# LUMII-Syslab/DiffusionSAT

Measured on NVIDIA B200. Metric: diffusion samples/sec, 3-SAT n=100, higher is better.
Workload: dtype f32

## Files before the change

### diffusionsat_b200/csrc/dsat_api.cu

```cuda
#include <cuda_runtime.h>
#include <math.h>
#include <stdint.h>
#include <stdio.h>
#include <stdlib.h>
#include <string.h>

#include <algorithm>
#include <string>
#include <type_traits>
#include <vector>

#include "../../include/dsat.h"
#include "../../include/dsat_debug.h"
#include "dsat_common.cuh"
#include "dsat_gemm_simt.cuh"
#include "dsat_message.cuh"
#include "dsat_spmm.cuh"
#include "dsat_graph_host.cuh"
#include "dsat_norm_head.cuh"
#include "dsat_hist.cuh"
#include "dsat_gemm_tc.cuh"
#include "dsat_mlp_fused.cuh"
#include "dsat_mlp_x3.cuh"

// ... 434 lines not shown
    cudaEventRecord(c->prof[c->prof_used].ev, c->stream);
    c->prof_used++;
}

int x3_pack_weights(dsat_ctx* c) {
    struct Cut { int op, col0, n; };
    const Cut cuts[12] = {
        {OP_V1, 0, c->HQ}, {OP_Q2, 0, c->Q}, {OP_V1, c->HQ, c->HL}, {OP_L2, 0, c->HL}, {OP_L3, 0, 2 * c->Q},
        {OP_C1, 0, c->HC}, {OP_C2, 0, c->Q + c->F}, {OP_U1, 0, c->HU}, {OP_U2, 0, c->HU}, {OP_U3, 0, c->F},
        {OP_O1, 0, c->HO}, {OP_O2, 0, DSAT_LOGIT_PAD}};
    for (int i = 0; i < 12; ++i) {
        const int op = cuts[i].op, K = c->ops[op].K, Nop = c->ops[op].N, n = cuts[i].n;
        const int K64 = (K + 63) / 64 * 64;
        std::vector<float> w((size_t)K * Nop);
        CK_CUDA(c, dsat_memcpy_sync(w.data(), c->ops[op].w.p, w.size() * sizeof(float), cudaMemcpyDeviceToHost));
        std::vector<__nv_bfloat16> wt((size_t)2 * n * K64, __float2bfloat16(0.f));
        for (int k = 0; k < K; ++k)
            for (int j = 0; j < n; ++j) {
                const float v = w[(size_t)k * Nop + cuts[i].col0 + j];
                const __nv_bfloat16 hi = __float2bfloat16(v);
                wt[(size_t)j * K64 + k] = hi;
                wt[(size_t)(n + j) * K64 + k] = __float2bfloat16(v - __bfloat162float(hi));
            }
        CK_CUDA(c, c->wx[i].alloc(wt.size()));
        CK_CUDA(c, dsat_memcpy_sync(c->wx[i].p, wt.data(), wt.size() * 2, cudaMemcpyHostToDevice));
        c->wx_k64[i] = K64; c->wx_n[i] = n;
    }
    return DSAT_OK;
}

enum { XQ = 0, XL1, XL2, XL3, XC, XU, XO };

int ensure_x3_buffers(dsat_ctx* c) {
    if (c->has_x3_buffers) return DSAT_OK;
    int rc = ensure_common_buffers(c);
    if (rc) return rc;
    const size_t Nt = (size_t)c->Nt, Mt = (size_t)c->Mt;
    const int F = c->F, Q = c->Q;
    CK_CUDA(c, c->VROWp.alloc(2 * Nt * c->ldv()));
    CK_CUDA(c, c->CROWp.alloc(2 * Mt * c->ldc()));
    CK_CUDA(c, c->SPREp.alloc(2 * Nt * F));
    CK_CUDA(c, c->H1p.alloc(2 * Nt * c->HL));
    CK_CUDA(c, c->H2p.alloc(2 * Nt * c->HL));
    CK_CUDA(c, cudaMemsetAsync(c->VROWp.p, 0, c->VROWp.count * 2, c->stream));
    CK_CUDA(c, cudaMemsetAsync(c->CROWp.p, 0, c->CROWp.count * 2, c->stream));
    struct L { int wi; int op; int bias_off; int epi; };
    auto build = [&](int which, const __nv_bfloat16* a_hi, size_t a_plane, long long rows, int k, int lda,
                     std::initializer_list<L> layers, int n_groups, int out_mode, void* out0, void* out1, int ld_out) -> bool {
        x3::X3Mlp& f = c->x3[which];
        f.ready = false;
        x3::X3Params& p = f.p;
        p.n_layers = (int)layers.size();
        p.rows = (int)rows;
        p.n_groups = n_groups;
        p.a_box_rows = (int)(rows < x3::BLOCK_M ? rows : x3::BLOCK_M);
        p.qmaps = Q;
        p.prof = nullptr;
        p.out_mode = out_mode; p.out0 = out0; p.out1 = out1; p.ld_out = ld_out;
        {
            const SkipInfo sk = skip_info(c);
            p.done = sk.done; p.chains_per_group = sk.chains_per_group;
            p.rows_per_chain = rows == c->Mt ? c->m : c->n;
        }
        f.pair_mode = which != XQ && which != XO;
        if (!tc::make_bf16_map(&f.map_a_hi, a_hi, rows, k, lda, p.a_box_rows)) return false;
        if (!tc::make_bf16_map(&f.map_a_lo, a_hi + a_plane, rows, k, lda, p.a_box_rows)) return false;
        int i = 0;
        for (const L& l : layers) {
            x3::X3Layer& ly = p.layer[i];
            const int n_total = c->wx_n[l.wi];
            ly.K = c->ops[l.op].K; ly.N = n_groups > 1 ? 256 : n_total; ly.n_total = n_total;
            ly.epi = l.epi; ly.w_lo_row = n_total; ly.bias = c->ops[l.op].b.p + l.bias_off;
            if (n_groups > 1 && n_total != 256 * n_groups) return false;
            ++i;
        }
        if (!x3::plan_x3(f)) return false;
        i = 0;
        for (const L& l : layers) {
            const int box = f.p.pair ? p.layer[i].N / 2 : p.layer[i].N;
            if (!tc::make_bf16_map(&f.map_w[i], c->wx[l.wi].p, 2 * c->wx_n[l.wi], c->wx_k64[l.wi], c->wx_k64[l.wi], box)) return false;
            ++i;
        }
        for (; i < x3::MAX_LAYERS; ++i) f.map_w[i] = f.map_w[0];
        if (getenv("DSAT_PLAN_LOG"))
            fprintf(stderr, "[dsat] x3 mlp %d: smem %d B, input ring %d, weight ring %d x %d B, epilogue warps %d, cta pair %d, groups %d\n",
                    which, f.smem_bytes, p.a_slots, p.w_slots, p.w_slot_bytes, p.epi_warps, p.pair, p.n_groups);
        return true;
    };
    const size_t vplane = Nt * c->ldv(), cplane = Mt * c->ldc(), splane = Nt * F, hplane = Nt * c->HL;
    bool ok = true;
    ok = ok && build(XQ, c->VROWp.p, vplane, c->Nt, F + DSAT_AUX_PAD, c->ldv(),
                     {{0, OP_V1, 0, tc::TC_LRELU}, {1, OP_Q2, 0, tc::TC_QUERY}}, 1, x3::OUT_F32, c->QS.p, nullptr, 3 * Q);
    const int lgroups = c->HL > 256 ? c->HL / 256 : 1;
    ok = ok && (c->HL <= 256 || c->HL % 256 == 0);
    ok = ok && build(XL1, c->VROWp.p, vplane, c->Nt, F + DSAT_AUX_PAD, c->ldv(),
                     {{2, OP_V1, c->HQ, tc::TC_LRELU}}, lgroups, x3::OUT_SPLIT, c->H1p.p, c->H1p.p + hplane, c->HL);
    ok = ok && build(XL2, c->H1p.p, hplane, c->Nt, c->HL, c->HL,
                     {{3, OP_L2, 0, tc::TC_LRELU}}, lgroups, x3::OUT_SPLIT, c->H2p.p, c->H2p.p + hplane, c->HL);
    const int l3groups = 2 * Q > 256 ? 2 * Q / 256 : 1;
    ok = ok && build(XL3, c->H2p.p, hplane, c->Nt, c->HL, c->HL,
                     {{4, OP_L3, 0, tc::TC_LINEAR}}, l3groups, x3::OUT_F32, c->LIT.p, nullptr, 2 * Q);
    if (Q + F <= 256 && c->HC <= 256)
        ok = ok && build(XC, c->CROWp.p, cplane, c->Mt, F + 2 * Q, c->ldc(),
                         {{5, OP_C1, 0, tc::TC_LRELU}, {6, OP_C2, 0, tc::TC_LINEAR}}, 1, x3::OUT_F32, c->COUT.p, nullptr, Q + F);
    else ok = false;
    if (c->HU <= 256)
        ok = ok && build(XU, c->VROWp.p, vplane, c->Nt, F + DSAT_AUX_PAD + 3 * Q, c->ldv(),
                         {{7, OP_U1, 0, tc::TC_LRELU}, {8, OP_U2, 0, tc::TC_LRELU}, {9, OP_U3, 0, tc::TC_LINEAR}}, 1, x3::OUT_F32,
                         c->UOUT.p, nullptr, F);
    else ok = false;
    ok = ok && build(XO, c->SPREp.p, splane, c->Nt, F, F,
                     {{10, OP_O1, 0, tc::TC_LRELU}, {11, OP_O2, 0, tc::TC_LINEAR}}, 1, x3::OUT_F32, c->LOGITS.p, nullptr, DSAT_LOGIT_PAD);
    c->x3_ready = ok;
    if (!ok) { c->err = "the fp32-accurate tensor-core path supports feature_maps = query_maps <= 128 (hidden widths <= 256 or 512)"; return DSAT_ERR_UNSUPPORTED; }
    c->has_x3_buffers = true;
    return DSAT_OK;
}

int run_x3(dsat_ctx* c, int which, int prof_class) {
    prof_mark(c, prof_class);
    CK_CUDA(c, x3::launch_x3(c->x3[which], c->device, c->sm_count, c->stream));
    c->launches++;
    return DSAT_OK;
}

int run_linear(dsat_ctx* c, int op, const float* A, int lda, float* Y, int ldy, long long rows, int epi) {
    prof_mark(c, op);
    LinearOp l;
    l.A = A; l.lda = lda; l.W = c->ops[op].w.p; l.ldw = c->ops[op].N; l.bias = c->ops[op].b.p;
    l.Y = Y; l.ldy = ldy; l.rows = (int)rows; l.K = c->ops[op].K; l.N = c->ops[op].N; l.epi = epi; l.qmaps = c->Q;
    CK_CUDA(c, launch_sgemm(l, c->stream));
    c->launches++;
    return DSAT_OK;
}

template <typename KernelLauncher>
int dispatch_width(dsat_ctx* c, int width, KernelLauncher&& fn) {
    switch (width) {
        case 64: fn(std::integral_constant<int, 2>()); break;
        case 128: fn(std::integral_constant<int, 4>()); break;
        case 256: fn(std::integral_constant<int, 8>()); break;
        default: c->err = "feature width must be 64, 128 or 256"; return DSAT_ERR_UNSUPPORTED;
    }
    return DSAT_OK;
}

struct LossScalars { float t, ts, norm_plus; };


float kl_host(float pa, float pb) {
    float qa = 1.0f - pa;
    float t1 = pa == 0.f ? 0.f : pa * (logf(pa) - logf(pb));
    float t2 = qa == 0.f ? 0.f : qa * (log1pf(-pa) - log1pf(-pb));
    return t1 + t2;
}
LossScalars loss_scalars(float noise_scale) {
    LossScalars s;
    s.t = powf(noise_scale, 0.5f);
    s.ts = fminf(s.t + 0.01f, 1.0f);
    float pa = 0.0f * (1.0f - s.ts) + s.ts / 2.0f;
    float pb = 0.0f * (1.0f - 1.0f) + 1.0f / 2.0f;
    s.norm_plus = kl_host(pa, pb) + 1e-4f;
    return s;
}

static inline bool use_tc(const dsat_ctx* c) { return c->precision == DSAT_BF16 || c->precision == DSAT_BF16_UNFUSED; }
static inline bool use_x3(const dsat_ctx* c) { return c->precision == DSAT_F32_TC; }
static inline float* vrow_f(dsat_ctx* c) { return c->precision == DSAT_F32 ? c->VROW.p : nullptr; }
static inline __nv_bfloat16* vrow_b(dsat_ctx* c) { return use_tc(c) ? c->VROWb.p : use_x3(c) ? c->VROWp.p : nullptr; }
// ... 1432 lines not shown
```

### diffusionsat_b200/csrc/dsat_gemm_tc.cuh

```cuda
#pragma once
#include <cuda.h>
#include "dsat_common.cuh"

namespace dsat {
namespace tc {

constexpr int BLOCK_M = 128;
constexpr int BLOCK_N = 256;
constexpr int BLOCK_K = 64;
constexpr int STAGES = 2;
constexpr int THREADS = 192;
constexpr int A_BYTES = BLOCK_M * BLOCK_K * 2;
constexpr int B_BYTES = BLOCK_N * BLOCK_K * 2;
constexpr int SMEM_BYTES = STAGES * (A_BYTES + B_BYTES) + 1024  + 256 ;

enum TcEpilogue : int { TC_LINEAR = 0, TC_LRELU = 1, TC_QUERY = 2 };

struct TcOut {
    void* ptr0; int ld0; int bf16_0;
    void* ptr1; int ld1; int bf16_1;
    int split;
};

__device__ __forceinline__ uint32_t smem_u32(const void* p) { return (uint32_t)__cvta_generic_to_shared(p); }
// ... 340 lines not shown
        }
    } else {
        const int quad = warp & 3;
        const size_t row = (size_t)row0 + quad * 32 + lane;
        mbar_wait(tmem_full_bar, 0);
        tcgen05_fence_after();
        for (int c = 0; c < bn; c += 32) {
            uint32_t raw[32];
            tmem_ld_32cols(tmem_base + ((uint32_t)(quad * 32) << 16) + (uint32_t)c, raw);
            if (row < (size_t)rows) {
                float v[32];
                const int col = n0 + c;
#pragma unroll
                for (int j = 0; j < 32; ++j) {
                    float x = __uint_as_float(raw[j]) + ((col + j < N) ? __ldg(bias + col + j) : 0.f);
                    if (epi == TC_LRELU) x = x > 0.f ? x : 0.2f * x;
                    v[j] = x;
                }
                const int valid = min(32, bn - c);
                if (valid == 32) {
                    store_chunk(out, row, col, v);
                    if (epi == TC_QUERY) {
                        float sp[32], sn[32];
#pragma unroll
                        for (int j = 0; j < 32; ++j) {
                            const float tail = __logf(1.0f + __expf(-fabsf(v[j])));
                            sp[j] = fmaxf(v[j], 0.f) + tail;
                            sn[j] = fmaxf(-v[j], 0.f) + tail;
                        }
                        store_chunk(out, row, col + qmaps, sp);
                        store_chunk(out, row, col + 2 * qmaps, sn);
                    }
                } else {
                    const bool second = out.ptr1 != nullptr && col >= out.split;
                    void* base = second ? out.ptr1 : out.ptr0;
                    const int ld = second ? out.ld1 : out.ld0;
                    const int cc = second ? col - out.split : col;
                    const int is_bf16 = second ? out.bf16_1 : out.bf16_0;
                    for (int j = 0; j < valid; ++j) {
                        if (is_bf16) reinterpret_cast<__nv_bfloat16*>(base)[row * ld + cc + j] = __float2bfloat16_rn(v[j]);
                        else reinterpret_cast<float*>(base)[row * ld + cc + j] = v[j];
                    }
                }
            }
        }
        tcgen05_fence_before();
    }
    __syncthreads();
    if (warp == 1) {
        tcgen05_fence_after();
        asm volatile("tcgen05.dealloc.cta_group::1.sync.aligned.b32 %0, %1;" ::"r"(tmem_base), "n"(BLOCK_N));
    }
}

typedef CUresult (*EncodeTiledFn)(CUtensorMap*, CUtensorMapDataType, cuuint32_t, void*, const cuuint64_t*,
                                  const cuuint64_t*, const cuuint32_t*, const cuuint32_t*, CUtensorMapInterleave,
                                  CUtensorMapSwizzle, CUtensorMapL2promotion, CUtensorMapFloatOOBfill);

inline EncodeTiledFn encode_tiled_fn() {
    static EncodeTiledFn fn = nullptr;
    if (!fn) {
        void* p = nullptr;
        cudaDriverEntryPointQueryResult q;
        if (cudaGetDriverEntryPoint("cuTensorMapEncodeTiled", &p, cudaEnableDefault, &q) == cudaSuccess &&
            q == cudaDriverEntryPointSuccess)
            fn = reinterpret_cast<EncodeTiledFn>(p);
    }
    return fn;
}

inline bool make_bf16_map(CUtensorMap* map, const void* base, long long rows, int cols, int ld, int box_rows) {
    EncodeTiledFn fn = encode_tiled_fn();
    if (!fn) return false;
    cuuint64_t dims[2] = {(cuuint64_t)cols, (cuuint64_t)rows};
    cuuint64_t strides[1] = {(cuuint64_t)ld * 2};
    cuuint32_t box[2] = {(cuuint32_t)BLOCK_K, (cuuint32_t)box_rows};
    cuuint32_t estr[2] = {1, 1};
    CUresult r = fn(map, CU_TENSOR_MAP_DATA_TYPE_BFLOAT16, 2, const_cast<void*>(base), dims, strides, box, estr,
                    CU_TENSOR_MAP_INTERLEAVE_NONE, CU_TENSOR_MAP_SWIZZLE_128B, CU_TENSOR_MAP_L2_PROMOTION_L2_256B,
                    CU_TENSOR_MAP_FLOAT_OOB_FILL_NONE);
    return r == CUDA_SUCCESS;
}

struct TcLinear {
    CUtensorMap map_a, map_b;
    const float* bias;
    TcOut out;
    int rows, K, N, epi, qmaps;
    int a_box_rows, b_box_rows;
};

inline cudaError_t configure_tc_device() {
    static PerDeviceOnce configured;
    if (configured.done()) return cudaSuccess;
    cudaError_t e = cudaFuncSetAttribute(tc_linear_kernel, cudaFuncAttributeMaxDynamicSharedMemorySize, SMEM_BYTES);
    if (e == cudaSuccess) configured.mark();
    return e;
}

inline cudaError_t launch_tc_linear(const TcLinear& op, cudaStream_t stream) {
    if (op.rows <= 0) return cudaSuccess;
    {
        cudaError_t e = configure_tc_device();
        if (e != cudaSuccess) return e;
    }
    const int n_tiles = ceil_div(op.N, BLOCK_N);
    const unsigned grid = (unsigned)(n_tiles * ceil_div(op.rows, BLOCK_M));
    tc_linear_kernel<<<grid, THREADS, SMEM_BYTES, stream>>>(op.map_a, op.map_b, op.bias, op.out, op.rows, op.K, op.N,
                                                             n_tiles, op.epi, op.qmaps, op.a_box_rows, op.b_box_rows);
    return cudaGetLastError();
}

}
}
```

### diffusionsat_b200/csrc/dsat_mlp_x3.cuh

```cuda
#pragma once
#include "dsat_mlp_fused.cuh"

namespace dsat {
namespace x3 {

constexpr int BLOCK_M = 128;
constexpr int BLOCK_K = 64;
constexpr int BLK_BYTES = BLOCK_M * BLOCK_K * 2;
constexpr int MAX_LAYERS = 3;
constexpr int MAX_RING = 12;
constexpr int TMEM_COLS = 512;
constexpr int STAGE_ROW = 128 + 16;
constexpr int SKIP_UNITS = 1024;
constexpr int SKIP_OFF = 512;
constexpr int BAR_BYTES = SKIP_OFF + SKIP_UNITS / 8;
static_assert((4 * MAX_RING + 6) * 8 + 4 <= SKIP_OFF, "x3 barriers overlap the early-exit bits");
constexpr int SMEM_LIMIT = 227 * 1024;

enum OutMode : int { OUT_F32 = 0, OUT_SPLIT = 1 };

struct X3Layer {
    int K, N;
    int epi;
    int w_lo_row;
    int bias_off;
    int n_total;
    const float* bias;
};

struct X3Params {
    int n_layers;
    X3Layer layer[MAX_LAYERS];
    int rows, n_tiles, n_groups, a_box_rows;
    int a_slots, w_slots, w_slot_bytes;
    int epi_warps, smem_pad, bias_total, qmaps, pair;
    int out_mode;
    void* out0; void* out1; int ld_out;
    long long* prof;
    const int* done; int rows_per_chain, chains_per_group;
};

__device__ __forceinline__ void split2(float v0, float v1, uint32_t& hi, uint32_t& lo) { split_bf16x2(v0, v1, hi, lo); }

struct Epi {
    uint32_t lane_addr, bl_addr, stage_addr;
    int N, epi, cpar, cstep, lane, qmaps, col0;
    size_t row_first; int rows_left;
    void* out0; void* out1; int ld_out, out_mode;
};

__device__ __forceinline__ void epi_hidden(const Epi& e, const uint32_t (&raw)[32], int c) {
    float v[32];
    fm::bias_act_chunk(raw, e.bl_addr + 4u * (uint32_t)c, e.epi == tc::TC_LRELU, v);
    uint32_t w[32];
#pragma unroll
    for (int i = 0; i < 16; ++i) split2(v[2 * i], v[2 * i + 1], w[i], w[16 + i]);
    fm::tmem_st_32cols(e.lane_addr + (uint32_t)c, w);
}

__device__ __forceinline__ void epi_final(const Epi& e, const uint32_t (&raw)[32], int c) {
    float v[32];
    fm::bias_act_chunk(raw, e.bl_addr + 4u * (uint32_t)c, e.epi == tc::TC_LRELU, v);
    const int valid = min(32, e.N - c);
    const int col = e.col0 + c;
    if (e.out_mode == OUT_SPLIT) {
        uint4 hi[4], lo[4];
#pragma unroll
        for (int q = 0; q < 4; ++q) {
            split2(v[8 * q], v[8 * q + 1], hi[q].x, lo[q].x);
            split2(v[8 * q + 2], v[8 * q + 3], hi[q].y, lo[q].y);
            split2(v[8 * q + 4], v[8 * q + 5], hi[q].z, lo[q].z);
            split2(v[8 * q + 6], v[8 * q + 7], hi[q].w, lo[q].w);
        }
        const size_t pitch = (size_t)e.ld_out * 2;
        fm::store_chunk_packed(e.stage_addr, STAGE_ROW, e.lane, hi, valid, reinterpret_cast<uint8_t*>(e.out0), pitch, e.row_first, e.rows_left, col);
        fm::store_chunk_packed(e.stage_addr, STAGE_ROW, e.lane, lo, valid, reinterpret_cast<uint8_t*>(e.out1), pitch, e.row_first, e.rows_left, col);
        return;
    }
    uint8_t* gbase = reinterpret_cast<uint8_t*>(e.out0);
    const size_t pitch = (size_t)e.ld_out * 4;
    fm::store_chunk_fast<false>(e.stage_addr, STAGE_ROW, e.lane, v, valid, gbase, pitch, e.row_first, e.rows_left, col);
    if (e.epi == tc::TC_QUERY) {
        float sp[32], sn[32];
#pragma unroll
        for (int i = 0; i < 32; ++i) {
            const float t = __logf(1.0f + __expf(-fabsf(v[i])));
            sp[i] = fmaxf(v[i], 0.f) + t;
            sn[i] = fmaxf(-v[i], 0.f) + t;
        }
        fm::store_chunk_fast<false>(e.stage_addr, STAGE_ROW, e.lane, sp, valid, gbase, pitch, e.row_first, e.rows_left, col + e.qmaps);
        fm::store_chunk_fast<false>(e.stage_addr, STAGE_ROW, e.lane, sn, valid, gbase, pitch, e.row_first, e.rows_left, col + 2 * e.qmaps);
    }
}

template <bool PAIR>
__global__ void __launch_bounds__(64 + 32 * 8, 1)
x3_mlp_kernel(const __grid_constant__ CUtensorMap map_a_hi, const __grid_constant__ CUtensorMap map_a_lo,
              const __grid_constant__ CUtensorMap map_w0, const __grid_constant__ CUtensorMap map_w1,
              const __grid_constant__ CUtensorMap map_w2, X3Params p) {
    using namespace tc;
    extern __shared__ __align__(1024) uint8_t smem_raw[];
    uint8_t* smem = reinterpret_cast<uint8_t*>((reinterpret_cast<uintptr_t>(smem_raw) + 1023) & ~(uintptr_t)1023);
    if ((int)(smem - smem_raw) > p.smem_pad) __trap();
    uint8_t* a_ring = smem;
    uint8_t* w_ring = a_ring + (size_t)p.a_slots * BLK_BYTES;
    uint8_t* stage_all = w_ring + (size_t)p.w_slots * p.w_slot_bytes;
    uint8_t* tail = stage_all + (size_t)p.epi_warps * 32 * STAGE_ROW;
    uint64_t* a_full = reinterpret_cast<uint64_t*>(tail);
    uint64_t* a_empty = a_full + MAX_RING;
    uint64_t* w_full = a_empty + MAX_RING;
    uint64_t* w_empty = w_full + MAX_RING;
    uint64_t* tmem_full = w_empty + MAX_RING;
    uint64_t* tmem_empty = tmem_full + 2;
    uint64_t* h_full = tmem_empty + 2;
    uint32_t* tmem_slot = reinterpret_cast<uint32_t*>(h_full + 2);
    float* bias_s = reinterpret_cast<float*>(tail + BAR_BYTES);

    const int warp = threadIdx.x >> 5, lane = threadIdx.x & 31;
    const int epi_threads = 32 * p.epi_warps;
    const CUtensorMap* map_w[MAX_LAYERS] = {&map_w0, &map_w1, &map_w2};
    const CUtensorMap* map_a[2] = {&map_a_hi, &map_a_lo};
    const uint32_t rank = PAIR ? cluster_rank() : 0u;
    const bool leader = rank == 0;
    constexpr int NC = PAIR ? 2 : 1;
    const bool timing = p.prof != nullptr && blockIdx.x == 0;

    if (threadIdx.x == 0) {
        for (int s = 0; s < MAX_RING; ++s) {
            mbar_init(&a_full[s], NC); mbar_init(&a_empty[s], 1);
            mbar_init(&w_full[s], NC); mbar_init(&w_empty[s], 1);
        }
        for (int b = 0; b < 2; ++b) { mbar_init(&tmem_full[b], 1); mbar_init(&tmem_empty[b], NC * p.epi_warps); }
        for (int h = 0; h < 2; ++h) mbar_init(&h_full[h], NC * p.epi_warps);
        asm volatile("fence.mbarrier_init.release.cluster;" ::: "memory");
        asm volatile("prefetch.tensormap [%0];" ::"l"(&map_a_hi) : "memory");
        asm volatile("prefetch.tensormap [%0];" ::"l"(&map_a_lo) : "memory");
        asm volatile("prefetch.tensormap [%0];" ::"l"(&map_w0) : "memory");
        asm volatile("prefetch.tensormap [%0];" ::"l"(&map_w1) : "memory");
        asm volatile("prefetch.tensormap [%0];" ::"l"(&map_w2) : "memory");
    }
    if (warp == 1) {
        if constexpr (PAIR) {
            asm volatile("tcgen05.alloc.cta_group::2.sync.aligned.shared::cta.b32 [%0], %1;" ::"r"(smem_u32(tmem_slot)), "n"(TMEM_COLS));
            asm volatile("tcgen05.relinquish_alloc_permit.cta_group::2.sync.aligned;");
        } else {
            asm volatile("tcgen05.alloc.cta_group::1.sync.aligned.shared::cta.b32 [%0], %1;" ::"r"(smem_u32(tmem_slot)), "n"(TMEM_COLS));
            asm volatile("tcgen05.relinquish_alloc_permit.cta_group::1.sync.aligned;");
        }
    }
    if (warp >= 2 && warp < 2 + p.epi_warps) {
        for (int l = 0; l < p.n_layers; ++l)
            for (int i = threadIdx.x - 64; i < p.layer[l].n_total; i += epi_threads) bias_s[p.layer[l].bias_off + i] = __ldg(p.layer[l].bias + i);
    }
    tcgen05_fence_before();
    __syncthreads();
    if constexpr (PAIR) cluster_sync_all();
    tcgen05_fence_after();
    const uint32_t tmem_base = *tmem_slot;
    const int L = p.n_layers, G = p.n_groups;
    auto at_leader = [&](uint64_t* bar) -> uint32_t { return PAIR ? mapa_rank(smem_u32(bar), 0) : smem_u32(bar); };
    const int unit0 = PAIR ? (int)(blockIdx.x >> 1) : (int)blockIdx.x;
    const int unit_stride = PAIR ? (int)(gridDim.x >> 1) : (int)gridDim.x;
    const int n_units = (PAIR ? (p.n_tiles + 1) / 2 : p.n_tiles) * G;
    const int nt = unit0 < n_units ? (n_units - unit0 + unit_stride - 1) / unit_stride : 0;
    auto tile_of = [&](int j) { const int u = (unit0 + j * unit_stride) / G; return PAIR ? 2 * u + (int)rank : u; };
    auto group_of = [&](int j) { return (unit0 + j * unit_stride) % G; };
    uint32_t* skip_bits = reinterpret_cast<uint32_t*>(tail + SKIP_OFF);
    const bool skipping = p.done != nullptr && nt <= SKIP_UNITS;
    if (skipping) {
        for (int base = 32 * warp; base < nt; base += (int)blockDim.x) {
            const int j = base + lane;
            bool all = false;
            if (j < nt) {
                const int u = (unit0 + j * unit_stride) / G;
                const int r0 = (PAIR ? 2 * u : u) * BLOCK_M;
                int r1 = r0 + (PAIR ? 2 * BLOCK_M : BLOCK_M);
                r1 = (r1 < p.rows ? r1 : p.rows) - 1;
                const int g0 = (r0 / p.rows_per_chain) / p.chains_per_group, g1 = (r1 / p.rows_per_chain) / p.chains_per_group;
                all = true;
                for (int g = g0; g <= g1 && all; ++g) all = __ldg(p.done + g) != 0;
            }
            const uint32_t bits = __ballot_sync(0xffffffffu, all);
// ... 71 lines not shown
                    }
                } else {
                    for (int k = 0; k < ksteps; ++k) {
                        if constexpr (PAIR) umma_bf16_elect_cg2(acc, da + (uint64_t)(2 * k), db + (uint64_t)(2 * k), idesc, (accum | (uint32_t)k) != 0);
                        else umma_bf16_elect(acc, da + (uint64_t)(2 * k), db + (uint64_t)(2 * k), idesc, (accum | (uint32_t)k) != 0);
                    }
                    if (free_bar) commit(free_bar);
                }
            };
#define X3_WAIT(acc_t, call) do { if (timing) { const long long t0__ = clock64(); call; acc_t += clock64() - t0__; } else { call; } } while (0)
            int jp = 0;
            for (int j = 0; j < nt; ++j) {
                if (unit_done(j)) continue;
                for (int l = 0; l < L; ++l) {
                    const int g = jp * L + l, buf = g & 1, use = g >> 1;
                    X3_WAIT(t_wait_acc, mbar_wait(&tmem_empty[buf], (uint32_t)((use & 1) ^ 1)));
                    if (g > 0 && (l > 0 ? l - 1 : L - 1) > 0)
                        X3_WAIT(t_wait_read, mbar_wait(&tmem_full[buf ^ 1], (uint32_t)(((g - 1) >> 1) & 1)));
                    const uint32_t h_par = (uint32_t)((jp * (L - 1) + (l - 1)) & 1);
                    tcgen05_fence_after();
                    const int K = p.layer[l].K, N = p.layer[l].N;
                    const int kbs = (K + BLOCK_K - 1) / BLOCK_K;
                    const uint32_t idesc = make_idesc_bf16(PAIR ? 2 * BLOCK_M : BLOCK_M, N);
                    const uint32_t acc = tmem_base + (uint32_t)(buf * 256);
                    const uint32_t hid = tmem_base + (uint32_t)((buf ^ 1) * 256);
                    for (int kb = 0; kb < kbs; ++kb) {
                        const int ksteps = min(BLOCK_K / 16, (K - kb * BLOCK_K + 15) / 16);
                        if (l == 0) {
                            const int as_hi = as;
                            const uint32_t ph_hi = aph;
                            if (++as == p.a_slots) { as = 0; aph ^= 1; }
                            const int as_lo = as;
                            const uint32_t ph_lo = aph;
                            if (++as == p.a_slots) { as = 0; aph ^= 1; }
                            X3_WAIT(t_wait_a, mbar_wait(&a_full[as_hi], ph_hi));
                            X3_WAIT(t_wait_a, mbar_wait(&a_full[as_lo], ph_lo));
                            const uint64_t da_hi = make_smem_desc_sw128(smem_u32(a_ring + (size_t)as_hi * BLK_BYTES));
                            const uint64_t da_lo = make_smem_desc_sw128(smem_u32(a_ring + (size_t)as_lo * BLK_BYTES));
                            X3_WAIT(t_wait_w, mbar_wait(&w_full[ws], wph));
                            uint64_t db = make_smem_desc_sw128(smem_u32(w_ring + (size_t)ws * p.w_slot_bytes));
                            kblock(acc, da_hi, db, idesc, kb != 0, ksteps, nullptr);
                            kblock(acc, da_lo, db, idesc, 1u, ksteps, &w_empty[ws]);
                            if (++ws == p.w_slots) { ws = 0; wph ^= 1; }
                            X3_WAIT(t_wait_w, mbar_wait(&w_full[ws], wph));
                            db = make_smem_desc_sw128(smem_u32(w_ring + (size_t)ws * p.w_slot_bytes));
                            kblock(acc, da_hi, db, idesc, 1u, ksteps, &w_empty[ws]);
                            if (++ws == p.w_slots) { ws = 0; wph ^= 1; }
                            commit(&a_empty[as_hi]); commit(&a_empty[as_lo]);
                        } else {
                            const uint32_t ta_hi = hid + (uint32_t)(kb * BLOCK_K), ta_lo = ta_hi + 16;
                            if ((kb & 1) == 0 && kb < 4) {
                                X3_WAIT(t_wait_h, mbar_wait(&h_full[kb >> 1], h_par));
                                tcgen05_fence_after();
                            }
                            X3_WAIT(t_wait_w, mbar_wait(&w_full[ws], wph));
                            uint64_t db = make_smem_desc_sw128(smem_u32(w_ring + (size_t)ws * p.w_slot_bytes));
                            kblock_ts(acc, ta_hi, db, idesc, kb != 0, ksteps, nullptr);
                            kblock_ts(acc, ta_lo, db, idesc, 1u, ksteps, &w_empty[ws]);
                            if (++ws == p.w_slots) { ws = 0; wph ^= 1; }
                            X3_WAIT(t_wait_w, mbar_wait(&w_full[ws], wph));
                            db = make_smem_desc_sw128(smem_u32(w_ring + (size_t)ws * p.w_slot_bytes));
                            kblock_ts(acc, ta_hi, db, idesc, 1u, ksteps, &w_empty[ws]);
                            if (++ws == p.w_slots) { ws = 0; wph ^= 1; }
                        }
                    }
                    commit(&tmem_full[buf]);
                }
                ++jp;
            }
#undef X3_WAIT
            if (timing && lane == 0) {
                p.prof[0] = clock64() - t_begin; p.prof[1] = t_wait_acc; p.prof[2] = t_wait_h; p.prof[3] = t_wait_a; p.prof[4] = t_wait_w;
                p.prof[8] = t_wait_read;
            }
        }
    } else if (warp < 2 + p.epi_warps) {
        const int quad = warp & 3;
        Epi e;
        e.lane = lane;
        e.cpar = (warp - 2) >> 2;
        e.cstep = 32 * (p.epi_warps >> 2);
        e.qmaps = p.qmaps;
        e.out0 = p.out0; e.out1 = p.out1; e.ld_out = p.ld_out; e.out_mode = p.out_mode;
        const uint32_t bias_addr0 = smem_u32(bias_s);
        e.stage_addr = smem_u32(stage_all) + (uint32_t)(warp - 2) * (32 * STAGE_ROW);
        long long t_wait_full = 0, t_hidden = 0, t_final = 0;
        int jp = -1;
        for (int j = 0; j < nt; ++j) {
            if (unit_done(j)) continue;
            ++jp;
            const int tile = tile_of(j), grp = group_of(j);
            DSAT_CHECK(tile >= 0 && (tile < p.n_tiles || (PAIR && tile == p.n_tiles)) && grp >= 0 && grp < G);
            e.row_first = (size_t)tile * BLOCK_M + quad * 32;
            e.rows_left = p.rows - (int)e.row_first;
            e.col0 = grp * 256;
            for (int l = 0; l < L; ++l) {
                const int g = jp * L + l, buf = g & 1, use = g >> 1;
                e.N = p.layer[l].N; e.epi = p.layer[l].epi;
                e.bl_addr = bias_addr0 + 4u * (uint32_t)(p.layer[l].bias_off + grp * 256);
                e.lane_addr = tmem_base + ((uint32_t)(quad * 32) << 16) + (uint32_t)(buf * 256);
                const long long t0 = timing ? clock64() : 0;
                mbar_wait(&tmem_full[buf], (uint32_t)(use & 1));
                tcgen05_fence_after();
                const long long t1 = timing ? clock64() : 0;
                const uint32_t empty_addr = at_leader(&tmem_empty[buf]);
                if (l + 1 < L) {
                    bool low_done = false;
                    auto release = [&](int h) {
                        fm::tmem_st_wait();
                        tcgen05_fence_before();
                        __syncwarp();
                        if (lane == 0) {
                            if (h == 1) fm::arrive_addr<PAIR>(empty_addr);
                            fm::arrive_addr<PAIR>(at_leader(&h_full[h]));
                        }
                    };
                    int c = 32 * e.cpar;
                    if (c < e.N) {
                        uint32_t ra[32], rb[32];
                        fm::tmem_ld_32cols_async(e.lane_addr + (uint32_t)c, ra);
#pragma unroll 1
                        while (true) {
                            fm::tmem_ld_wait(ra);
                            const int c1 = c + e.cstep;
                            if (c1 < e.N) fm::tmem_ld_32cols_async(e.lane_addr + (uint32_t)c1, rb);
                            epi_hidden(e, ra, c);
                            if (!low_done && c1 >= 128) { release(0); low_done = true; }
                            if (c1 >= e.N) break;
                            fm::tmem_ld_wait(rb);
                            c = c1 + e.cstep;
                            if (c < e.N) fm::tmem_ld_32cols_async(e.lane_addr + (uint32_t)c, ra);
                            epi_hidden(e, rb, c1);
                            if (!low_done && c >= 128) { release(0); low_done = true; }
                            if (c >= e.N) break;
                        }
                    }
                    if (!low_done) release(0);
                    release(1);
                    if (timing) t_hidden += clock64() - t1;
                } else {
                    bool released = false;
#pragma unroll 1
                    for (int c = 32 * e.cpar; c < e.N; c += e.cstep) {
                        uint32_t ra[32];
                        fm::tmem_ld_32cols_async(e.lane_addr + (uint32_t)c, ra);
                        fm::tmem_ld_wait(ra);
                        if (c + e.cstep >= e.N) {
                            tcgen05_fence_before();
                            fm::warp_arrive<PAIR>(empty_addr, lane);
                            released = true;
                        }
                        epi_final(e, ra, c);
                    }
                    if (!released) { tcgen05_fence_before(); fm::warp_arrive<PAIR>(empty_addr, lane); }
                    if (timing) t_final += clock64() - t1;
                }
                if (timing) t_wait_full += t1 - t0;
            }
        }
        if (timing && warp == 2 && lane == 0) { p.prof[5] = t_wait_full; p.prof[6] = t_hidden; p.prof[7] = t_final; }
    }
    tcgen05_fence_before();
    __syncthreads();
    if constexpr (PAIR) cluster_sync_all();
    if (warp == 1) {
        tcgen05_fence_after();
        if constexpr (PAIR) asm volatile("tcgen05.dealloc.cta_group::2.sync.aligned.b32 %0, %1;" ::"r"(tmem_base), "n"(TMEM_COLS));
        else asm volatile("tcgen05.dealloc.cta_group::1.sync.aligned.b32 %0, %1;" ::"r"(tmem_base), "n"(TMEM_COLS));
    }
}

struct X3Mlp {
    CUtensorMap map_a_hi, map_a_lo;
    CUtensorMap map_w[MAX_LAYERS];
    X3Params p;
    int smem_bytes = 0;
    bool pair_mode = false;
    bool ready = false;
};

inline bool plan_x3(X3Mlp& f) {
    X3Params& p = f.p;
    const int pad = fm::dyn_smem_pad();
    p.smem_pad = pad;
    int bias_total = 0, max_n = 0;
    bool pair = f.pair_mode && p.rows > BLOCK_M;
    for (int l = 0; l < p.n_layers; ++l) {
        X3Layer& ly = p.layer[l];
        if (ly.N > 256 || ly.N % 16 || ly.K % 16) return false;
        if (l > 0 && ly.K > p.layer[l - 1].N) return false;
        ly.bias_off = bias_total;
        bias_total += (ly.n_total + 31) / 32 * 32;
        max_n = max(max_n, ly.N);
    }
    if (p.n_groups > 1 && p.n_layers != 1) return false;
    p.pair = pair ? 1 : 0;
    p.bias_total = bias_total;
    p.n_tiles = ceil_div(p.rows, BLOCK_M);
    p.w_slot_bytes = ((pair ? max_n / 2 : max_n) * BLOCK_K * 2 + 1023) / 1024 * 1024;
    for (int ew : {8, 4}) {
        const int fixed = pad + ew * 32 * STAGE_ROW + BAR_BYTES + bias_total * 4;
        int avail = SMEM_LIMIT - fixed;
        int a = 2, w = 2;
        if (avail < a * BLK_BYTES + w * p.w_slot_bytes) continue;
        avail -= a * BLK_BYTES + w * p.w_slot_bytes;
        while (true) {
            bool grew = false;
            if (a <= w && a < MAX_RING && avail >= BLK_BYTES) { ++a; avail -= BLK_BYTES; grew = true; }
            else if (w < MAX_RING && avail >= p.w_slot_bytes) { ++w; avail -= p.w_slot_bytes; grew = true; }
            else if (a < MAX_RING && avail >= BLK_BYTES) { ++a; avail -= BLK_BYTES; grew = true; }
            if (!grew) break;
        }
        p.a_slots = a; p.w_slots = w; p.epi_warps = ew;
        f.smem_bytes = fixed + a * BLK_BYTES + w * p.w_slot_bytes;
        f.ready = true;
        return true;
    }
    return false;
}

inline cudaError_t configure_x3_device(int) {
    static PerDeviceOnce configured;
    if (configured.done()) return cudaSuccess;
    cudaError_t e = cudaFuncSetAttribute(x3_mlp_kernel<false>, cudaFuncAttributeMaxDynamicSharedMemorySize, SMEM_LIMIT);
    if (e == cudaSuccess) e = cudaFuncSetAttribute(x3_mlp_kernel<true>, cudaFuncAttributeMaxDynamicSharedMemorySize, SMEM_LIMIT);
    if (e == cudaSuccess) configured.mark();
    return e;
}

inline cudaError_t launch_x3(const X3Mlp& f, int device, int sm_count, cudaStream_t stream) {
    if (f.p.rows <= 0) return cudaSuccess;
    cudaError_t e = configure_x3_device(device);
    if (e != cudaSuccess) return e;
    const unsigned threads = 64 + 32 * f.p.epi_warps;
    if (f.p.pair) {
        const int n_units = (f.p.n_tiles + 1) / 2 * f.p.n_groups;
        const int pairs = n_units < sm_count / 2 ? n_units : sm_count / 2;
        cudaLaunchConfig_t cfg = {};
        cfg.gridDim = dim3(2 * pairs); cfg.blockDim = dim3(threads); cfg.dynamicSmemBytes = (size_t)f.smem_bytes; cfg.stream = stream;
        cudaLaunchAttribute attr[1];
        attr[0].id = cudaLaunchAttributeClusterDimension;
        attr[0].val.clusterDim.x = 2; attr[0].val.clusterDim.y = 1; attr[0].val.clusterDim.z = 1;
        cfg.attrs = attr; cfg.numAttrs = 1;
        return cudaLaunchKernelEx(&cfg, x3_mlp_kernel<true>, f.map_a_hi, f.map_a_lo, f.map_w[0], f.map_w[1], f.map_w[2], f.p);
    }
    const int n_units = f.p.n_tiles * f.p.n_groups;
    const unsigned grid = (unsigned)(n_units < sm_count ? n_units : sm_count);
    x3_mlp_kernel<false><<<grid, threads, f.smem_bytes, stream>>>(f.map_a_hi, f.map_a_lo, f.map_w[0], f.map_w[1], f.map_w[2], f.p);
    return cudaGetLastError();
}

}
}
```

### diffusionsat_b200/csrc/dsat_norm_head.cuh

```cuda
#pragma once
#include "dsat_common.cuh"
#include "dsat_message.cuh"

namespace dsat {

template <int V>
__device__ __forceinline__ int lane_col(int lane, int i) {
    if constexpr (V == 2) return lane * 2 + i;
    else return (i >> 2) * 128 + lane * 4 + (i & 3);
}

constexpr int PN_WARPS = 8;
#ifndef PN_BF16_CTAS
#define PN_BF16_CTAS 4
#endif
constexpr int PN_UNROLL = 4;

template <int V, typename TS, typename TX>
__global__ void __launch_bounds__(PN_WARPS * 32)
pairnorm_kernel(const int* __restrict__ seg, int n_graphs_unit, int rows_per_chain, int total_graphs,
                const TS* __restrict__ SRC, int ld_src, int src_off,
                TX* __restrict__ STATE, int ld_state,
                TX* __restrict__ PRE, int ld_pre,
                __nv_bfloat16* STATE_HI = nullptr, size_t state_plane = 0,
// ... 17 lines not shown
            for (; r + (PN_UNROLL - 1) * PN_WARPS < r1; r += PN_UNROLL * PN_WARPS) {
                LaneVec<V> x[PN_UNROLL];
#pragma unroll
                for (int u = 0; u < PN_UNROLL; ++u)
                    x[u] = lane_load_t<V, TS>(SRC + (r + u * PN_WARPS) * ld_src + src_off, lane);
#pragma unroll
                for (int u = 0; u < PN_UNROLL; ++u)
#pragma unroll
                    for (int i = 0; i < V; ++i) sum.v[i] += x[u].v[i] * wgt;
            }
            for (; r < r1; r += PN_WARPS) {
                LaneVec<V> x = lane_load_t<V, TS>(SRC + r * ld_src + src_off, lane);
#pragma unroll
                for (int i = 0; i < V; ++i) sum.v[i] += x.v[i] * wgt;
            }
        }
#pragma unroll
        for (int i = 0; i < V; ++i) red[warp][lane_col<V>(lane, i)] = sum.v[i];
        __syncthreads();
        for (int col = tid; col < F; col += PN_WARPS * 32) {
            float s = 0.f;
#pragma unroll
            for (int w = 0; w < PN_WARPS; ++w) s += red[w][col];
            mean_s[col] = s;
        }
        __syncthreads();
        LaneVec<V> mean;
#pragma unroll
        for (int i = 0; i < V; ++i) mean.v[i] = mean_s[lane_col<V>(lane, i)];
        auto finish_row = [&](size_t r, LaneVec<V> x, const LaneVec<V>& old) {
            float ss = 0.f;
#pragma unroll
            for (int i = 0; i < V; ++i) { x.v[i] -= mean.v[i]; ss += x.v[i] * x.v[i]; }
            ss = warp_sum(ss);
            const float inv = rsqrtf(ss / (float)F + 1.0e-6f);
            LaneVec<V> nw, carried;
#pragma unroll
            for (int i = 0; i < V; ++i) {
                nw.v[i] = __fadd_rn(__fmul_rn(x.v[i] * inv, 0.25f), __fmul_rn(0.1f, old.v[i]));
                carried.v[i] = __fadd_rn(__fmul_rn(nw.v[i], 0.2f), __fmul_rn(nw.v[i], 0.8f));
            }
            if (STATE_HI) {
                if (PRE_HI) lane_store_split<V>(PRE_HI + r * ld_pre, pre_plane, lane, nw);
                lane_store_split<V>(STATE_HI + r * ld_state, state_plane, lane, carried);
                return;
            }
            if (PRE) lane_store_t<V, TX>(PRE + r * ld_pre, lane, nw);
            lane_store_t<V, TX>(STATE + r * ld_state, lane, carried);
        };
        auto load_old = [&](size_t r) {
            return STATE_HI ? lane_load_split_rw<V>(STATE_HI + r * ld_state, state_plane, lane)
                            : lane_load_rw_t<V, TX>(STATE + r * ld_state, lane);
        };
        {
            size_t r = r0 + warp;
            for (; r + (PN_UNROLL - 1) * PN_WARPS < r1; r += PN_UNROLL * PN_WARPS) {
                LaneVec<V> x[PN_UNROLL], old[PN_UNROLL];
#pragma unroll
                for (int u = 0; u < PN_UNROLL; ++u) {
                    x[u] = lane_load_t<V, TS>(SRC + (r + u * PN_WARPS) * ld_src + src_off, lane);
                    old[u] = load_old(r + u * PN_WARPS);
                }
#pragma unroll
                for (int u = 0; u < PN_UNROLL; ++u) finish_row(r + u * PN_WARPS, x[u], old[u]);
            }
            for (; r < r1; r += PN_WARPS) {
                LaneVec<V> x = lane_load_t<V, TS>(SRC + r * ld_src + src_off, lane);
                LaneVec<V> old = load_old(r);
                finish_row(r, x, old);
            }
        }
        __syncthreads();
    }
}

template <int V>
__global__ void __launch_bounds__(1024)
pairnorm_smem_kernel(const int* __restrict__ seg, int n_graphs_unit, int rows_per_chain, int total_graphs,
                     const float* __restrict__ SRC, int ld_src, int src_off,
                     __nv_bfloat16* STATE_HI, size_t state_plane, int ld_state,
                     __nv_bfloat16* __restrict__ PRE_HI, size_t pre_plane, int ld_pre, SkipInfo skip = SkipInfo{nullptr, 1}) {
    constexpr int F = 32 * V;
    constexpr int PPR = F / 4;
    extern __shared__ __align__(16) uint8_t pn_smem[];
    float* mean_s = reinterpret_cast<float*>(pn_smem);
    float* part = mean_s + F;
    const int tid = threadIdx.x, lane = tid & 31, warp = tid >> 5, nwarps = blockDim.x >> 5;
    const int groups = blockDim.x / F > 0 ? blockDim.x / F : 1;
    float* rows = part + groups * F;
    for (int gid = blockIdx.x; gid < total_graphs; gid += gridDim.x) {
        const int chain = gid / n_graphs_unit, lg = gid % n_graphs_unit;
        if (chain_done(skip, chain)) continue;
        const size_t base = (size_t)chain * rows_per_chain;
        const size_t r0 = base + __ldg(seg + lg);
        const int nrows = __ldg(seg + lg + 1) - __ldg(seg + lg);
        const float wgt = 1.0f / (float)nrows;
        DSAT_CHECK(nrows > 0 && r0 + nrows <= (size_t)(chain + 1) * rows_per_chain);
        for (int i = tid; i < nrows * PPR; i += blockDim.x) {
            const int r = i / PPR, k = i % PPR;
            cp_async16(rows + (size_t)r * F + 4 * k, SRC + (r0 + r) * ld_src + src_off + 4 * k);
        }
        cp_async_wait_all();
        __syncthreads();
        if (tid < groups * F) {
            const int col = tid % F, grp = tid / F;
            float s = 0.f;
            for (int r = grp; r < nrows; r += groups) s += rows[(size_t)r * F + col] * wgt;
            part[grp * F + col] = s;
        }
        __syncthreads();
        if (tid < F) {
            float s = 0.f;
            for (int k = 0; k < groups; ++k) s += part[k * F + tid];
            mean_s[tid] = s;
        }
        __syncthreads();
        LaneVec<V> mean;
#pragma unroll
        for (int i = 0; i < V; ++i) mean.v[i] = mean_s[lane_col<V>(lane, i)];
        auto finish_row = [&](int r, const LaneVec<V>& old) {
            LaneVec<V> x = lane_load_rw<V>(rows + (size_t)r * F, lane);
            float ss = 0.f;
#pragma unroll
            for (int i = 0; i < V; ++i) { x.v[i] -= mean.v[i]; ss += x.v[i] * x.v[i]; }
            ss = warp_sum(ss);
            const float inv = rsqrtf(ss / (float)F + 1.0e-6f);
            LaneVec<V> nw, carried;
#pragma unroll
            for (int i = 0; i < V; ++i) {
                nw.v[i] = __fadd_rn(__fmul_rn(x.v[i] * inv, 0.25f), __fmul_rn(0.1f, old.v[i]));
                carried.v[i] = __fadd_rn(__fmul_rn(nw.v[i], 0.2f), __fmul_rn(nw.v[i], 0.8f));
            }
            if (PRE_HI) lane_store_split<V>(PRE_HI + (r0 + r) * ld_pre, pre_plane, lane, nw);
            lane_store_split<V>(STATE_HI + (r0 + r) * ld_state, state_plane, lane, carried);
        };
        int r = warp;
        for (; r + (PN_UNROLL - 1) * nwarps < nrows; r += PN_UNROLL * nwarps) {
            LaneVec<V> old[PN_UNROLL];
#pragma unroll
            for (int u = 0; u < PN_UNROLL; ++u) old[u] = lane_load_split_rw<V>(STATE_HI + (r0 + r + u * nwarps) * ld_state, state_plane, lane);
#pragma unroll
            for (int u = 0; u < PN_UNROLL; ++u) finish_row(r + u * nwarps, old[u]);
        }
        for (; r < nrows; r += nwarps) finish_row(r, lane_load_split_rw<V>(STATE_HI + (r0 + r) * ld_state, state_plane, lane));
        __syncthreads();
    }
}

__device__ __forceinline__ float bernoulli_kl(float pa, float pb) {
    const float qa = 1.0f - pa;
    const float t1 = pa == 0.f ? 0.f : pa * (logf(pa) - logf(pb));
    const float t2 = qa == 0.f ? 0.f : qa * (log1pf(-pa) - log1pf(-pb));
    return t1 + t2;
}

template <int F>
__global__ void __launch_bounds__(PN_WARPS * 32, PN_BF16_CTAS)
pairnorm_bf16_kernel(const int* __restrict__ seg, int n_graphs_unit, int rows_per_chain, int total_graphs,
                     const __nv_bfloat16* __restrict__ SRC, int ld_src, int src_off,
                     __nv_bfloat16* __restrict__ STATE, int ld_state,
                     __nv_bfloat16* __restrict__ PRE, int ld_pre, SkipInfo skip = SkipInfo{nullptr, 1}) {
    constexpr int LPR = F / 8, RPW = 32 / LPR, GROUP = PN_WARPS * RPW;
    __shared__ float red[PN_WARPS][F];
    __shared__ float mean_s[F];
    const int tid = threadIdx.x, lane = tid & 31, warp = tid >> 5;
    const int sub = lane / LPR, li = lane % LPR;
    for (int gid = blockIdx.x; gid < total_graphs; gid += gridDim.x) {
        const int chain = gid / n_graphs_unit, lg = gid % n_graphs_unit;
        if (chain_done(skip, chain)) continue;
        const size_t base = (size_t)chain * rows_per_chain;
        const size_t r0 = base + __ldg(seg + lg), r1 = base + __ldg(seg + lg + 1);
        const float wgt = 1.0f / (float)(r1 - r0);
        float sum[8];
#pragma unroll
        for (int i = 0; i < 8; ++i) sum[i] = 0.f;
        for (size_t rb = r0 + warp * RPW; rb < r1; rb += (size_t)PN_UNROLL * GROUP) {
            const size_t r = rb + sub;
            uint4 x[PN_UNROLL];
#pragma unroll
            for (int u = 0; u < PN_UNROLL; ++u) {
                const size_t rr = r + (size_t)u * GROUP;
                x[u] = make_uint4(0u, 0u, 0u, 0u);
                if (rr < r1) x[u] = __ldg(reinterpret_cast<const uint4*>(SRC + rr * ld_src + src_off) + li);
            }
#pragma unroll
            for (int u = 0; u < PN_UNROLL; ++u) {
                float v[8];
                unpack8(x[u], v);
#pragma unroll
                for (int i = 0; i < 8; ++i) sum[i] += v[i] * wgt;
            }
        }
#pragma unroll
        for (int off = LPR; off < 32; off <<= 1)
#pragma unroll
            for (int i = 0; i < 8; ++i) sum[i] += __shfl_xor_sync(0xffffffffu, sum[i], off);
        if (sub == 0) {
#pragma unroll
            for (int i = 0; i < 8; ++i) red[warp][li * 8 + i] = sum[i];
        }
        __syncthreads();
        for (int col = tid; col < F; col += PN_WARPS * 32) {
            float s = 0.f;
#pragma unroll
            for (int w = 0; w < PN_WARPS; ++w) s += red[w][col];
            mean_s[col] = s;
        }
        __syncthreads();
        float mean[8];
#pragma unroll
        for (int i = 0; i < 8; ++i) mean[i] = mean_s[li * 8 + i];
        for (size_t rb = r0 + warp * RPW; rb < r1; rb += (size_t)PN_UNROLL * GROUP) {
            const size_t r = rb + sub;
            uint4 x[PN_UNROLL], old[PN_UNROLL];
#pragma unroll
            for (int u = 0; u < PN_UNROLL; ++u) {
                const size_t rr = r + (size_t)u * GROUP;
                x[u] = make_uint4(0u, 0u, 0u, 0u); old[u] = x[u];
                if (rr < r1) {
                    x[u] = __ldg(reinterpret_cast<const uint4*>(SRC + rr * ld_src + src_off) + li);
                    old[u] = reinterpret_cast<const uint4*>(STATE + rr * ld_state)[li];
                }
            }
#pragma unroll
            for (int u = 0; u < PN_UNROLL; ++u) {
                const size_t rr = r + (size_t)u * GROUP;
                float v[8], o[8], nw[8], carried[8];
                unpack8(x[u], v);
// ... 333 lines not shown
```

Before: 737.0.

## Use TMA tensor stores for x3 MLP f32 outputs and prefetch next graph in pairnorm

The x3 MLP final epilogue can now write f32 output chunks through a swizzled shared-memory stage followed by TMA bulk tensor stores, replacing per-thread global stores when the output width is a multiple of 32. Separately, the pairnorm kernel now software-pipelines across graphs: while it finishes rows of the current graph, each warp stages rows of the next graph into shared memory with cp.async, removing the barrier-separated load phase at the start of each graph. It also lowers the unroll factor for wide features to reduce register pressure. The risks are the bulk-group waits serialising the epilogue, the TMA stage layout not fitting the existing shared-memory plan, and subtle races in reusing the row buffer.

```diff
diff --git a/diffusionsat_b200/csrc/dsat_api.cu b/diffusionsat_b200/csrc/dsat_api.cu
--- a/diffusionsat_b200/csrc/dsat_api.cu
+++ b/diffusionsat_b200/csrc/dsat_api.cu
@@ -540,9 +540,12 @@
             ++i;
         }
         for (; i < x3::MAX_LAYERS; ++i) f.map_w[i] = f.map_w[0];
+        p.tma_out = out_mode == x3::OUT_F32 && p.layer[p.n_layers - 1].N % 32 == 0;
+        if (p.tma_out && !tc::make_f32_out_map(&f.map_out, out0, rows, ld_out, ld_out)) return false;
+        if (!p.tma_out) f.map_out = f.map_a_hi;
         if (getenv("DSAT_PLAN_LOG"))
-            fprintf(stderr, "[dsat] x3 mlp %d: smem %d B, input ring %d, weight ring %d x %d B, epilogue warps %d, cta pair %d, groups %d\n",
-                    which, f.smem_bytes, p.a_slots, p.w_slots, p.w_slot_bytes, p.epi_warps, p.pair, p.n_groups);
+            fprintf(stderr, "[dsat] x3 mlp %d: smem %d B, input ring %d, weight ring %d x %d B, epilogue warps %d, cta pair %d, groups %d, tma store %d\n",
+                    which, f.smem_bytes, p.a_slots, p.w_slots, p.w_slot_bytes, p.epi_warps, p.pair, p.n_groups, p.tma_out);
         return true;
     };
     const size_t vplane = Nt * c->ldv(), cplane = Mt * c->ldc(), splane = Nt * F, hplane = Nt * c->HL;
diff --git a/diffusionsat_b200/csrc/dsat_gemm_tc.cuh b/diffusionsat_b200/csrc/dsat_gemm_tc.cuh
--- a/diffusionsat_b200/csrc/dsat_gemm_tc.cuh
+++ b/diffusionsat_b200/csrc/dsat_gemm_tc.cuh
@@ -446,6 +446,18 @@
     return r == CUDA_SUCCESS;
 }
 
+inline bool make_f32_out_map(CUtensorMap* map, void* base, long long rows, int cols, int ld) {
+    EncodeTiledFn fn = encode_tiled_fn();
+    if (!fn) return false;
+    cuuint64_t dims[2] = {(cuuint64_t)cols, (cuuint64_t)rows};
+    cuuint64_t strides[1] = {(cuuint64_t)ld * 4};
+    cuuint32_t box[2] = {32, 32};
+    cuuint32_t estr[2] = {1, 1};
+    CUresult r = fn(map, CU_TENSOR_MAP_DATA_TYPE_FLOAT32, 2, base, dims, strides, box, estr, CU_TENSOR_MAP_INTERLEAVE_NONE,
+                    CU_TENSOR_MAP_SWIZZLE_128B, CU_TENSOR_MAP_L2_PROMOTION_NONE, CU_TENSOR_MAP_FLOAT_OOB_FILL_NONE);
+    return r == CUDA_SUCCESS;
+}
+
 struct TcLinear {
     CUtensorMap map_a, map_b;
     const float* bias;
diff --git a/diffusionsat_b200/csrc/dsat_mlp_x3.cuh b/diffusionsat_b200/csrc/dsat_mlp_x3.cuh
--- a/diffusionsat_b200/csrc/dsat_mlp_x3.cuh
+++ b/diffusionsat_b200/csrc/dsat_mlp_x3.cuh
@@ -11,6 +11,7 @@
 constexpr int MAX_RING = 12;
 constexpr int TMEM_COLS = 512;
 constexpr int STAGE_ROW = 128 + 16;
+constexpr int TMA_STAGE = 32 * 128;
 constexpr int SKIP_UNITS = 1024;
 constexpr int SKIP_OFF = 512;
 constexpr int BAR_BYTES = SKIP_OFF + SKIP_UNITS / 8;
@@ -35,6 +36,7 @@
     int a_slots, w_slots, w_slot_bytes;
     int epi_warps, smem_pad, bias_total, qmaps, pair;
     int out_mode;
+    int tma_out;
     void* out0; void* out1; int ld_out;
     long long* prof;
     const int* done; int rows_per_chain, chains_per_group;
@@ -47,7 +49,28 @@
     int N, epi, cpar, cstep, lane, qmaps, col0;
     size_t row_first; int rows_left;
     void* out0; void* out1; int ld_out, out_mode;
+    const CUtensorMap* map_out;
 };
+
+__device__ __forceinline__ void store_chunk_tma(const Epi& e, const float (&v)[32], int col) {
+    if (e.lane == 0) asm volatile("cp.async.bulk.wait_group.read 0;" ::: "memory");
+    __syncwarp();
+    const uint32_t row = e.stage_addr + (uint32_t)e.lane * 128u;
+#pragma unroll
+    for (int q = 0; q < 8; ++q) {
+        uint4 w;
+        w.x = __float_as_uint(v[4 * q]); w.y = __float_as_uint(v[4 * q + 1]);
+        w.z = __float_as_uint(v[4 * q + 2]); w.w = __float_as_uint(v[4 * q + 3]);
+        fm::sts128(row + (uint32_t)((q ^ (e.lane & 7)) << 4), w);
+    }
+    asm volatile("fence.proxy.async.shared::cta;" ::: "memory");
+    __syncwarp();
+    if (e.lane == 0) {
+        asm volatile("cp.async.bulk.tensor.2d.global.shared::cta.bulk_group [%0, {%1, %2}], [%3];"
+                     ::"l"(e.map_out), "r"(col), "r"((int)e.row_first), "r"(e.stage_addr) : "memory");
+        asm volatile("cp.async.bulk.commit_group;" ::: "memory");
+    }
+}
 
 __device__ __forceinline__ void epi_hidden(const Epi& e, const uint32_t (&raw)[32], int c) {
     float v[32];
@@ -79,7 +102,8 @@
     }
     uint8_t* gbase = reinterpret_cast<uint8_t*>(e.out0);
     const size_t pitch = (size_t)e.ld_out * 4;
-    fm::store_chunk_fast<false>(e.stage_addr, STAGE_ROW, e.lane, v, valid, gbase, pitch, e.row_first, e.rows_left, col);
+    if (e.map_out) store_chunk_tma(e, v, col);
+    else fm::store_chunk_fast<false>(e.stage_addr, STAGE_ROW, e.lane, v, valid, gbase, pitch, e.row_first, e.rows_left, col);
     if (e.epi == tc::TC_QUERY) {
         float sp[32], sn[32];
 #pragma unroll
@@ -88,8 +112,13 @@
             sp[i] = fmaxf(v[i], 0.f) + t;
             sn[i] = fmaxf(-v[i], 0.f) + t;
         }
-        fm::store_chunk_fast<false>(e.stage_addr, STAGE_ROW, e.lane, sp, valid, gbase, pitch, e.row_first, e.rows_left, col + e.qmaps);
-        fm::store_chunk_fast<false>(e.stage_addr, STAGE_ROW, e.lane, sn, valid, gbase, pitch, e.row_first, e.rows_left, col + 2 * e.qmaps);
+        if (e.map_out) {
+            store_chunk_tma(e, sp, col + e.qmaps);
+            store_chunk_tma(e, sn, col + 2 * e.qmaps);
+        } else {
+            fm::store_chunk_fast<false>(e.stage_addr, STAGE_ROW, e.lane, sp, valid, gbase, pitch, e.row_first, e.rows_left, col + e.qmaps);
+            fm::store_chunk_fast<false>(e.stage_addr, STAGE_ROW, e.lane, sn, valid, gbase, pitch, e.row_first, e.rows_left, col + 2 * e.qmaps);
+        }
     }
 }
 
@@ -97,7 +126,7 @@
 __global__ void __launch_bounds__(64 + 32 * 8, 1)
 x3_mlp_kernel(const __grid_constant__ CUtensorMap map_a_hi, const __grid_constant__ CUtensorMap map_a_lo,
               const __grid_constant__ CUtensorMap map_w0, const __grid_constant__ CUtensorMap map_w1,
-              const __grid_constant__ CUtensorMap map_w2, X3Params p) {
+              const __grid_constant__ CUtensorMap map_w2, const __grid_constant__ CUtensorMap map_out, X3Params p) {
     using namespace tc;
     extern __shared__ __align__(1024) uint8_t smem_raw[];
     uint8_t* smem = reinterpret_cast<uint8_t*>((reinterpret_cast<uintptr_t>(smem_raw) + 1023) & ~(uintptr_t)1023);
@@ -335,8 +364,9 @@
         e.cstep = 32 * (p.epi_warps >> 2);
         e.qmaps = p.qmaps;
         e.out0 = p.out0; e.out1 = p.out1; e.ld_out = p.ld_out; e.out_mode = p.out_mode;
+        e.map_out = p.tma_out ? &map_out : nullptr;
         const uint32_t bias_addr0 = smem_u32(bias_s);
-        e.stage_addr = smem_u32(stage_all) + (uint32_t)(warp - 2) * (32 * STAGE_ROW);
+        e.stage_addr = smem_u32(stage_all) + (uint32_t)(warp - 2) * (p.tma_out ? TMA_STAGE : 32 * STAGE_ROW);
         long long t_wait_full = 0, t_hidden = 0, t_final = 0;
         int jp = -1;
         for (int j = 0; j < nt; ++j) {
@@ -412,6 +442,7 @@
             }
         }
         if (timing && warp == 2 && lane == 0) { p.prof[5] = t_wait_full; p.prof[6] = t_hidden; p.prof[7] = t_final; }
+        if (e.map_out && lane == 0) asm volatile("cp.async.bulk.wait_group 0;" ::: "memory");
     }
     tcgen05_fence_before();
     __syncthreads();
@@ -426,6 +457,7 @@
 struct X3Mlp {
     CUtensorMap map_a_hi, map_a_lo;
     CUtensorMap map_w[MAX_LAYERS];
+    CUtensorMap map_out;
     X3Params p;
     int smem_bytes = 0;
     bool pair_mode = false;
@@ -495,11 +527,11 @@
         attr[0].id = cudaLaunchAttributeClusterDimension;
         attr[0].val.clusterDim.x = 2; attr[0].val.clusterDim.y = 1; attr[0].val.clusterDim.z = 1;
         cfg.attrs = attr; cfg.numAttrs = 1;
-        return cudaLaunchKernelEx(&cfg, x3_mlp_kernel<true>, f.map_a_hi, f.map_a_lo, f.map_w[0], f.map_w[1], f.map_w[2], f.p);
+        return cudaLaunchKernelEx(&cfg, x3_mlp_kernel<true>, f.map_a_hi, f.map_a_lo, f.map_w[0], f.map_w[1], f.map_w[2], f.map_out, f.p);
     }
     const int n_units = f.p.n_tiles * f.p.n_groups;
     const unsigned grid = (unsigned)(n_units < sm_count ? n_units : sm_count);
-    x3_mlp_kernel<false><<<grid, threads, f.smem_bytes, stream>>>(f.map_a_hi, f.map_a_lo, f.map_w[0], f.map_w[1], f.map_w[2], f.p);
+    x3_mlp_kernel<false><<<grid, threads, f.smem_bytes, stream>>>(f.map_a_hi, f.map_a_lo, f.map_w[0], f.map_w[1], f.map_w[2], f.map_out, f.p);
     return cudaGetLastError();
 }
 
diff --git a/diffusionsat_b200/csrc/dsat_norm_head.cuh b/diffusionsat_b200/csrc/dsat_norm_head.cuh
--- a/diffusionsat_b200/csrc/dsat_norm_head.cuh
+++ b/diffusionsat_b200/csrc/dsat_norm_head.cuh
@@ -123,24 +123,43 @@
                      __nv_bfloat16* __restrict__ PRE_HI, size_t pre_plane, int ld_pre, SkipInfo skip = SkipInfo{nullptr, 1}) {
     constexpr int F = 32 * V;
     constexpr int PPR = F / 4;
+    constexpr int U = V >= 8 ? 2 : PN_UNROLL;
     extern __shared__ __align__(16) uint8_t pn_smem[];
     float* mean_s = reinterpret_cast<float*>(pn_smem);
     float* part = mean_s + F;
     const int tid = threadIdx.x, lane = tid & 31, warp = tid >> 5, nwarps = blockDim.x >> 5;
     const int groups = blockDim.x / F > 0 ? blockDim.x / F : 1;
     float* rows = part + groups * F;
-    for (int gid = blockIdx.x; gid < total_graphs; gid += gridDim.x) {
-        const int chain = gid / n_graphs_unit, lg = gid % n_graphs_unit;
-        if (chain_done(skip, chain)) continue;
-        const size_t base = (size_t)chain * rows_per_chain;
-        const size_t r0 = base + __ldg(seg + lg);
-        const int nrows = __ldg(seg + lg + 1) - __ldg(seg + lg);
-        const float wgt = 1.0f / (float)nrows;
+    auto next_graph = [&](int g) {
+        for (g += gridDim.x; g < total_graphs && chain_done(skip, g / n_graphs_unit); g += gridDim.x) {}
+        return g;
+    };
+    auto graph_rows = [&](int g, size_t& r0, int& nrows) {
+        const int chain = g / n_graphs_unit, lg = g % n_graphs_unit;
+        r0 = (size_t)chain * rows_per_chain + __ldg(seg + lg);
+        nrows = __ldg(seg + lg + 1) - __ldg(seg + lg);
         DSAT_CHECK(nrows > 0 && r0 + nrows <= (size_t)(chain + 1) * rows_per_chain);
+    };
+    auto stage_row = [&](const float* g_src, int r) {
+        for (int k = lane; k < PPR; k += 32) cp_async16(rows + (size_t)r * F + 4 * k, g_src + (size_t)r * ld_src + 4 * k);
+    };
+    int gid = next_graph((int)blockIdx.x - (int)gridDim.x);
+    size_t r0 = 0;
+    int nrows = 0;
+    if (gid < total_graphs) {
+        graph_rows(gid, r0, nrows);
         for (int i = tid; i < nrows * PPR; i += blockDim.x) {
             const int r = i / PPR, k = i % PPR;
             cp_async16(rows + (size_t)r * F + 4 * k, SRC + (r0 + r) * ld_src + src_off + 4 * k);
         }
+    }
+    while (gid < total_graphs) {
+        const int nxt = next_graph(gid);
+        size_t nx_r0 = 0;
+        int nx_rows = 0;
+        if (nxt < total_graphs) graph_rows(nxt, nx_r0, nx_rows);
+        const float* nx_src = SRC + nx_r0 * ld_src + src_off;
+        const float wgt = 1.0f / (float)nrows;
         cp_async_wait_all();
         __syncthreads();
         if (tid < groups * F) {
@@ -159,6 +178,7 @@
         LaneVec<V> mean;
 #pragma unroll
         for (int i = 0; i < V; ++i) mean.v[i] = mean_s[lane_col<V>(lane, i)];
+        for (int r = nrows + warp; r < nx_rows; r += nwarps) stage_row(nx_src, r);
         auto finish_row = [&](int r, const LaneVec<V>& old) {
             LaneVec<V> x = lane_load_rw<V>(rows + (size_t)r * F, lane);
             float ss = 0.f;
@@ -176,15 +196,23 @@
             lane_store_split<V>(STATE_HI + (r0 + r) * ld_state, state_plane, lane, carried);
         };
         int r = warp;
-        for (; r + (PN_UNROLL - 1) * nwarps < nrows; r += PN_UNROLL * nwarps) {
-            LaneVec<V> old[PN_UNROLL];
-#pragma unroll
-            for (int u = 0; u < PN_UNROLL; ++u) old[u] = lane_load_split_rw<V>(STATE_HI + (r0 + r + u * nwarps) * ld_state, state_plane, lane);
-#pragma unroll
-            for (int u = 0; u < PN_UNROLL; ++u) finish_row(r + u * nwarps, old[u]);
-        }
-        for (; r < nrows; r += nwarps) finish_row(r, lane_load_split_rw<V>(STATE_HI + (r0 + r) * ld_state, state_plane, lane));
-        __syncthreads();
+        for (; r + (U - 1) * nwarps < nrows; r += U * nwarps) {
+            LaneVec<V> old[U];
+#pragma unroll
+            for (int u = 0; u < U; ++u) old[u] = lane_load_split_rw<V>(STATE_HI + (r0 + r + u * nwarps) * ld_state, state_plane, lane);
+#pragma unroll
+            for (int u = 0; u < U; ++u) finish_row(r + u * nwarps, old[u]);
+            __syncwarp();
+#pragma unroll
+            for (int u = 0; u < U; ++u)
+                if (r + u * nwarps < nx_rows) stage_row(nx_src, r + u * nwarps);
+        }
+        for (; r < nrows; r += nwarps) {
+            finish_row(r, lane_load_split_rw<V>(STATE_HI + (r0 + r) * ld_state, state_plane, lane));
+            __syncwarp();
+            if (r < nx_rows) stage_row(nx_src, r);
+        }
+        gid = nxt; r0 = nx_r0; nrows = nx_rows;
     }
 }
 
```

New measurement: 752.0, median of 6. 1.02x the previous value.
